# bytedance/monolith

Measured on AMD Instinct MI355X. Metric: embedding lookups+updates/sec at 1B ids x dim64, Zipf(1.2) batch=65536, higher is better.
Workload: dtype f32

## Files before the change

monolith_amd/csrc/mhte_step_kernels.h:

```cpp
#ifndef MHTE_STEP_KERNELS_H_
#define MHTE_STEP_KERNELS_H_

#include "mhte_kernels.h"

namespace mhte {

constexpr int kRdBlock = 1024;
constexpr int kRdLds = 2048;
constexpr int kRdStride = kRdLds + 1;
constexpr int kRdMaxBlocks = 64;
constexpr int kLongRun = kLightMax;
constexpr int kStepLightMax = 32;
constexpr int kMaxLongRuns = 16;
constexpr uint32_t kItemTarget = 256;
constexpr uint32_t kSpecSlackRows = 32;
#ifndef MHTE_BWD_OCC
#define MHTE_BWD_OCC 5
#endif
constexpr int kBwdBlocksPerCu = MHTE_BWD_OCC;

__device__ __forceinline__ void lds_barrier() {
  asm volatile("s_waitcnt lgkmcnt(0)\n\ts_barrier" ::: "memory");
}
__device__ __forceinline__ void lds_wave_sync() {
// ... 423 lines not shown
  uint32_t v = vt[ls];
  int left = kRdLds;
  while (k != id) {
    if (--left == 0) return 0u;
    ls = (ls + 1u) & (kRdLds - 1);
    k = kt[ls];
    v = vt[ls];
  }
  return v;
}

__device__ __forceinline__ uint32_t rd_find_run_opt(const RunView& d, uint32_t b, int64_t id) {
  const int64_t* kt = d.btab_key + size_t(b) * kRdStride;
  const uint32_t* vt = d.btab_val + size_t(b) * kRdStride;
  if (id == kEmptyKey) return run_cnt(vt[kRdLds]) ? vt[kRdLds] : 0u;
  uint32_t ls = rd_home(id);
  int64_t k = kt[ls];
  uint32_t v = vt[ls];
  int left = kRdLds;
  while (k != id) {
    if (k == kEmptyKey || --left == 0) return 0u;
    ls = (ls + 1u) & (kRdLds - 1);
    k = kt[ls];
    v = vt[ls];
  }
  return v;
}

__device__ __forceinline__ uint32_t rd_item_blocks(uint32_t c, uint32_t target) {
  uint32_t nbk = 64;
  const uint64_t lim = uint64_t(target) * 64 * (c > 2 * target ? 1 : 2);
  while (nbk > 1 && uint64_t(c) * nbk > lim) nbk >>= 1;
  return nbk;
}

constexpr int kBuildSlotsPerLane = 4;

constexpr int kMaxShards = 64;
__device__ __forceinline__ uint32_t shard_of_id(int64_t id, uint32_t nshards) {
  const int64_t m = id % int64_t(nshards);
  return uint32_t(m < 0 ? m + int64_t(nshards) : m);
}
struct PackCtl {
  int64_t* send_ids;
  const unsigned long long* peer_win;
  unsigned long long peer_ids_off;
  uint32_t* slot_off;
  uint32_t* flags;
  uint32_t world, ids_block, rows_block;
  uint32_t hdr_word;
  uint32_t cap, id_off, row_off, dim;
};

__device__ __forceinline__ void rd_emit_items(const RunView& d, int64_t id, uint32_t hu, uint32_t c,
                                              uint32_t hrow, uint32_t hspec, unsigned long long hloc,
                                              int lane) {
  const uint32_t val = (uint32_t(lane) < d.nblk) ? rd_find_run_opt(d, uint32_t(lane), id) : 0u;
  const unsigned long long bm = __ballot(val != 0u);
  const uint32_t nbk = rd_item_blocks(c, d.item_target);
  const uint32_t b0 = uint32_t(lane) & ~(nbk - 1u);
  const unsigned long long rmask = (nbk == 64 ? ~0ull : ((1ull << nbk) - 1ull)) << b0;
  const bool leader = (uint32_t(lane) == b0) && (bm & rmask) != 0ull;
  const unsigned long long lm = __ballot(leader);
  const uint32_t nitems = __popcll(lm);
  uint32_t w0 = 0;
  if (lane == 0) w0 = atomicAdd(&d.ctr[2], nitems);
  w0 = __shfl(w0, 0);
  const uint32_t k = __popcll(lm & ((1ull << b0) - 1ull));
  if (leader) {
    ItemHdr hd;
    hd.id = id;
    hd.u = hu;
    hd.meta = b0 | (nbk << 8) | (k << 16) | (nitems << 24);
    hd.row = hrow;
    hd.spec = hspec;
    hd.loc = hloc;
    d.item_hdr[w0 + k] = hd;
  }
  if ((bm & rmask) != 0ull) d.item_runs[size_t(w0 + k) * 64 + (uint32_t(lane) - b0)] = val;
}

constexpr unsigned long long kNoLoc = ~0ull;
struct __attribute__((aligned(16))) URec {
  int64_t id;
  uint32_t cnt;
  uint32_t pos;
  uint32_t slot;
  uint32_t row;
  unsigned long long loc;
};
struct ProbeOut {
  URec* urec;
  uint32_t reserve;
};

template <bool PACK = false, bool PROBE = false>
__device__ __forceinline__ void rd_build_role(const RunView& d, uint32_t light_max, uint32_t bid,
                                              uint32_t nblocks, const PackCtl* pc = nullptr,
                                              const TableView* tv = nullptr, ProbeOut po = ProbeOut{}) {
  constexpr int Q = kBuildSlotsPerLane;
  __shared__ uint32_t sh_tot[4];
  __shared__ uint32_t sh_base;
  __shared__ uint32_t sh_mtot[PROBE ? 4 : 1];
  __shared__ uint32_t sh_mbase;
  __shared__ uint8_t sh_stage[PROBE ? 4 * 256 : 4];
  __shared__ uint32_t sh_pc[PACK ? kMaxShards : 1], sh_pb[PACK ? kMaxShards : 1];
  const uint32_t t = threadIdx.x;
  const int lane = t & 63;
  const uint32_t nslots = d.cap_mask + 2u;
  for (uint32_t bb = bid * (256u * Q); bb < nslots; bb += nblocks * (256u * Q)) {
    const uint32_t base = bb + (t >> 6) * (64u * Q);
    int64_t key[Q];
    uint32_t cnt[Q], pos[Q];
    unsigned long long occ[Q];
    uint32_t total = 0;
    if (PACK) {
      if (t < pc->world) sh_pc[t] = 0;
      lds_barrier();
    }
#pragma unroll
    for (int q = 0; q < Q; ++q) {
      const uint32_t sl = base + q * 64 + lane;
      const bool in = sl < nslots;
      const RdSlot sv = d.hs[in ? sl : 0u];
      key[q] = in ? sv.key : kEmptyKey;
      cnt[q] = in ? uint32_t(sv.cp) : 0u;
      pos[q] = in ? uint32_t(sv.cp >> 32) : 0u;
    }
#pragma unroll
    for (int q = 0; q < Q; ++q) {
      const uint32_t sl = base + q * 64 + lane;
      const bool o = key[q] != kEmptyKey;
// ... 14 lines not shown
          prank[q] = atomicAdd(&sh_pc[pown[q]], 1u);
        }
      }
    }
    if (lane == 0) sh_tot[t >> 6] = total;
    lds_barrier();
    if (t == 0) {
      const uint32_t all = sh_tot[0] + sh_tot[1] + sh_tot[2] + sh_tot[3];
      sh_base = all ? atomicAdd(&d.ctr[0], all) : 0u;
    }
    if (PACK && t < pc->world) {
      const uint32_t c = sh_pc[t];
      sh_pb[t] = c ? uint32_t(atomicAdd(reinterpret_cast<unsigned long long*>(
                                            pc->send_ids + size_t(t) * pc->ids_block + pc->hdr_word),
                                        static_cast<unsigned long long>(c)))
                   : 0u;
    }
    lds_barrier();
    uint32_t k0 = sh_base;
    for (uint32_t w2 = 0; w2 < (t >> 6); ++w2) k0 += sh_tot[w2];
    const uint32_t kw0 = k0;
    const uint32_t wg_max = max(max(sh_tot[0], sh_tot[1]), max(sh_tot[2], sh_tot[3]));
    lds_barrier();
    uint32_t kq[Q];
#pragma unroll
    for (int q = 0; q < Q; ++q) {
      kq[q] = k0 + uint32_t(__popcll(occ[q] & ((1ull << lane) - 1ull)));
      k0 += uint32_t(__popcll(occ[q]));
      if ((occ[q] >> lane) & 1ull) {
        d.uids[kq[q]] = key[q];
        d.uslot[kq[q]] = base + q * 64 + lane;
        d.ucnt[kq[q]] = cnt[q];
        d.upos[kq[q]] = pos[q];
        if (PACK) {
          const uint32_t sl = sh_pb[pown[q]] + prank[q];
          if (sl < pc->cap) {
            if (pc->peer_win)
              reinterpret_cast<int64_t*>(pc->peer_win[pown[q]] + pc->peer_ids_off)[pc->id_off + sl] = key[q];
            else
              pc->send_ids[size_t(pown[q]) * pc->ids_block + pc->id_off + sl] = key[q];
            pc->slot_off[kq[q]] = pown[q] * pc->rows_block + pc->row_off + sl * pc->dim;
          } else {
            pc->slot_off[kq[q]] = 0xffffffffu;
            atomicOr(pc->flags, 1u);
          }
        }
      }
    }
    if (!PROBE) {
#pragma unroll
      for (int q = 0; q < Q; ++q) {
        unsigned long long hm = occ[q] & __ballot(cnt[q] > light_max);
        while (hm) {
          const int src = __ffsll(static_cast<long long>(hm)) - 1;
          hm &= hm - 1ull;
          rd_emit_items(d, __shfl(key[q], src), __shfl(kq[q], src), __shfl(cnt[q], src), kNoRow, kNoRow, 0ull,
                        lane);
        }
      }
    } else {
      typedef long long i64x2 __attribute__((ext_vector_type(2)));
      typedef unsigned int u32x4 __attribute__((ext_vector_type(4)));
      uint8_t* const stg = sh_stage + (t >> 6) * 256u;
      uint32_t run = 0;
#pragma unroll
      for (int q = 0; q < Q; ++q) {
        if ((occ[q] >> lane) & 1ull) stg[run + uint32_t(__popcll(occ[q] & ((1ull << lane) - 1ull)))] = uint8_t(q * 64 + lane);
        run += uint32_t(__popcll(occ[q]));
      }
      lds_wave_sync();
#pragma unroll 1
      for (uint32_t r0 = 0; r0 < wg_max; r0 += 64) {
        const uint32_t r = r0 + uint32_t(lane);
        const bool have = r < run;
        const uint32_t src = have ? uint32_t(stg[r]) : 0u;
        const int sl = int(src & 63u);
        int64_t kid = 0;
        uint32_t kc = 0, kp = 0;
#pragma unroll
        for (int q = 0; q < Q; ++q) {
          const int64_t kk = __shfl(key[q], sl);
          const uint32_t cc = __shfl(cnt[q], sl), pp = __shfl(pos[q], sl);
          if (int(src >> 6) == q) {
            kid = kk;
            kc = cc;
            kp = pp;
          }
        }
        const bool act = have && kid != kEmptyKey;
        const int64_t pid = act ? kid : 0;
        const uint64_t hv = hash_key(pid);
        const uint64_t i1 = index_hash(tv->hp, hv);
        const uint64_t i2 = alt_index(tv->hp, partial_key(hv), i1);
        const GBucket* b1 = global_bucket(tv->buckets + i1);
        const GBucket* b2 = global_bucket(tv->buckets + i2);
        const i64x2 k0a = *(const MHTE_GLOBAL i64x2*)(&b1->key[0]);
        const i64x2 k0b = *(const MHTE_GLOBAL i64x2*)(&b1->key[2]);
        const i64x2 k1a = *(const MHTE_GLOBAL i64x2*)(&b2->key[0]);
        const i64x2 k1b = *(const MHTE_GLOBAL i64x2*)(&b2->key[2]);
        const u32x4 r0v = *(const MHTE_GLOBAL u32x4*)(&b1->row[0]);
        const u32x4 r1v = *(const MHTE_GLOBAL u32x4*)(&b2->row[0]);
        int fs = -1;
        uint32_t fr = kNoRow;
        if (k1b.y == pid) { fs = 7; fr = r1v.w; }
        if (k1b.x == pid) { fs = 6; fr = r1v.z; }
        if (k1a.y == pid) { fs = 5; fr = r1v.y; }
        if (k1a.x == pid) { fs = 4; fr = r1v.x; }
        if (k0b.y == pid) { fs = 3; fr = r0v.w; }
        if (k0b.x == pid) { fs = 2; fr = r0v.z; }
        if (k0a.y == pid) { fs = 1; fr = r0v.y; }
        if (k0a.x == pid) { fs = 0; fr = r0v.x; }
        const bool found = act && fs >= 0 && fr != kNoRow;
        const bool miss = act && fs < 0;
        uint32_t spec = kNoRow;
        if (po.reserve) {
          const unsigned long long mm = __ballot(miss);
          if (lane == 0) sh_mtot[t >> 6] = uint32_t(__popcll(mm));
          lds_barrier();
          if (t == 0) {
            const unsigned long long all = sh_mtot[0] + sh_mtot[1] + sh_mtot[2] + sh_mtot[3];
            sh_mbase = all ? uint32_t(atomicAdd(&tv->ctr->alloc, (all << 32) | all)) : 0u;
            if (all) {
              atomicAdd(&tv->ctr->reserved, uint32_t(all));
              atomicAdd(&d.ctr[3], uint32_t(all));
            }
          }
          lds_barrier();
          uint32_t m0 = sh_mbase;
          for (uint32_t w2 = 0; w2 < (t >> 6); ++w2) m0 += sh_mtot[w2];
          lds_barrier();
          if (miss) spec = m0 + uint32_t(__popcll(mm & ((1ull << lane) - 1ull)));
        }
        const unsigned long long floc = found ? (((fs & 4) ? i2 : i1) << 2) | uint64_t(fs & 3) : kNoLoc;
        const uint32_t frow = found ? fr : spec;
        if (have) {
          URec rec;
          rec.id = kid;
          rec.cnt = kc;
          rec.pos = kp;
          rec.slot = base + (src >> 6) * 64u + (src & 63u);
          rec.row = frow;
          rec.loc = floc;
          po.urec[kw0 + r] = rec;
        }
        unsigned long long hm = __ballot(have && kc > light_max);
        while (hm) {
          const int s2 = __ffsll(static_cast<long long>(hm)) - 1;
          hm &= hm - 1ull;
          const unsigned long long hl = __shfl(floc, s2);
          rd_emit_items(d, __shfl(kid, s2), kw0 + r0 + uint32_t(s2), __shfl(kc, s2),
                        hl != kNoLoc ? __shfl(frow, s2) : kNoRow, hl != kNoLoc ? kNoRow : __shfl(frow, s2),
                        hl != kNoLoc ? hl : 0ull, lane);
        }
      }
    }
  }
  if (t == 0) {
    if (atomicAdd(&d.ctr[1], 1u) == nblocks - 1) *d.n_unique = atomicAdd(&d.ctr[0], 0u);
  }
}

__global__ __launch_bounds__(256) void rd_build_kernel(RunView d, uint32_t light_max) {
  rd_build_role(d, light_max, blockIdx.x, gridDim.x);
}
__global__ __launch_bounds__(256) void rd_build_probe_kernel(RunView d, uint32_t light_max, TableView tv,
                                                             ProbeOut po) {
  rd_build_role<false, true>(d, light_max, blockIdx.x, gridDim.x, nullptr, &tv, po);
}
__global__ __launch_bounds__(256) void rd_probe_kernel(RunView d, TableView tv, ProbeOut po, uint32_t n_max,
                                                       uint32_t light_max) {
  typedef long long i64x2 __attribute__((ext_vector_type(2)));
  typedef unsigned int u32x4 __attribute__((ext_vector_type(4)));
  __shared__ uint32_t sh_mtot[4];
  __shared__ uint32_t sh_mbase;
  const uint32_t t = threadIdx.x;
  const int lane = t & 63;
  const uint32_t nu = min(n_max, d.ctr[0]);
#pragma unroll 1
  for (uint32_t u0 = blockIdx.x * 256u; u0 < nu; u0 += gridDim.x * 256u) {
    const uint32_t u = u0 + t;
    const bool have = u < nu;
    const uint32_t us = have ? u : 0u;
    const int64_t kid = d.uids[us];
    const bool act = have && kid != kEmptyKey;
    const int64_t pid = act ? kid : 0;
    const uint64_t hv = hash_key(pid);
    const uint64_t i1 = index_hash(tv.hp, hv);
    const uint64_t i2 = alt_index(tv.hp, partial_key(hv), i1);
    const GBucket* b1 = global_bucket(tv.buckets + i1);
    const GBucket* b2 = global_bucket(tv.buckets + i2);
    const i64x2 k0a = *(const MHTE_GLOBAL i64x2*)(&b1->key[0]);
    const i64x2 k0b = *(const MHTE_GLOBAL i64x2*)(&b1->key[2]);
    const i64x2 k1a = *(const MHTE_GLOBAL i64x2*)(&b2->key[0]);
    const i64x2 k1b = *(const MHTE_GLOBAL i64x2*)(&b2->key[2]);
    const u32x4 r0v = *(const MHTE_GLOBAL u32x4*)(&b1->row[0]);
    const u32x4 r1v = *(const MHTE_GLOBAL u32x4*)(&b2->row[0]);
    URec rec;
    rec.id = kid;
    rec.cnt = d.ucnt[us];
    rec.pos = d.upos[us];
    rec.slot = d.uslot[us];
    int fs = -1;
    uint32_t fr = kNoRow;
    if (k1b.y == pid) { fs = 7; fr = r1v.w; }
    if (k1b.x == pid) { fs = 6; fr = r1v.z; }
// ... 99 lines not shown
  float* st2 = st1 + sd.dim;
  const bool has1 = sd.opt == kOptAdagrad || sd.opt == kOptFtrl;
  const bool has2 = sd.opt == kOptFtrl;
  Vec<VEC> s2;
  vec_zero(s2);
  if (is_new) {
    const SegDesc si = seg_for_init(sd);
#pragma unroll
    for (int c = 0; c < VEC; ++c) {
      r.w.v[c] = init_weight(si, rp + e + c);
      r.s1.v[c] = sd.p[0];
    }
  } else if (has2) {
    s2.load(st2);
  }
  if (sd.opt == kOptSgd) {
    const float slr = opaque_f(lr);
#pragma unroll
    for (int c = 0; c < VEC; ++c) r.w.v[c] = sgd_step(r.w.v[c], g.v[c], slr);
  } else if (sd.opt == kOptAdagrad) {
    const float alr = opaque_f(lr), wd = opaque_f(sd.p[1]);
    if (MHTE_AVX_FORM(sd)) {
#pragma unroll
      for (int c = 0; c < VEC; ++c)
        adagrad_step_avx(r.w.v[c], r.s1.v[c], g.v[c], alr, wd, uint32_t(le + c) < (uint32_t(sd.dim) & ~7u));
    } else {
#pragma unroll
      for (int c = 0; c < VEC; ++c) adagrad_step(r.w.v[c], r.s1.v[c], g.v[c], alr, wd);
    }
  } else {
    const float flr = opaque_f(lr), beta = opaque_f(sd.p[1]), l1 = opaque_f(sd.p[2]), l2 = opaque_f(sd.p[3]);
#pragma unroll
    for (int c = 0; c < VEC; ++c) ftrl_step(r.w.v[c], r.s1.v[c], s2.v[c], g.v[c], flr, beta, l1, l2);
  }
  row_store<VEC>(rp + e, r.w);
  if (has1) row_store<VEC>(st1, r.s1);
  if (has2) row_store<VEC>(st2, s2);
}

__device__ __forceinline__ void defer_id(const TableView& tv, uint32_t* pending, uint32_t u) {
  auto* ctr = tv.ctr;
#ifndef MHTE_NO_ANTIHOIST
  asm volatile("" : "+v"(ctr));
#endif
  pending[atomicAdd(&ctr->n_pending, 1u)] = u;
}

template <int G>
struct Probe {
  GBucket* b;
  int64_t k;
  uint32_t row;
};
template <int G>
__device__ __forceinline__ Probe<G> probe_issue(const TableView& tv, int64_t id, bool valid, int j) {
  const uint64_t hv = hash_key(id);
  const uint64_t i1 = index_hash(tv.hp, hv);
  const uint64_t i2 = alt_index(tv.hp, partial_key(hv), i1);
  Probe<G> p;
  p.b = global_bucket(tv.buckets + ((j < 4) ? i1 : i2));
  p.k = kEmptyKey;
  p.row = kNoRow;
  if (valid && id != kEmptyKey && j < 8) {
    p.k = p.b->key[j & 3];
    p.row = p.b->row[j & 3];
  }
  return p;
}

template <int VEC>
__device__ __forceinline__ void sum_list_lds(const float* __restrict__ grads, uint32_t dim,
                                             uint32_t e, bool ev, const uint32_t* pos, uint32_t c,
                                             Vec<VEC>& acc) {
#pragma unroll 1
  for (uint32_t q = 0; q < c; q += 8) {
    uint32_t ps[8];
#pragma unroll
    for (int t = 0; t < 8; ++t) ps[t] = (q + t < c) ? pos[q + t] : 0u;
    Vec<VEC> v[8];
#pragma unroll
    for (int t = 0; t < 8; ++t) vec_zero(v[t]);
#pragma unroll
    for (int t = 0; t < 8; ++t)
      if (q + t < c && ev) v[t].load(grads + int64_t(ps[t]) * dim + e);
#pragma unroll
    for (int t = 0; t < 8; ++t)
      if (q + t < c && ev) vec_add(acc, v[t]);
  }
}

template <int G>
struct UpsertFlight {
  unsigned long long cas_old;
  uint64_t specm;
  int owner, pick;
  bool found, need, special, deferred;
};

template <int G>
__device__ __forceinline__ UpsertFlight<G> upsert_issue(const TableView& tv, GBucket* b, int64_t id,
                                                        bool valid, int64_t k, int lane,
                                                        uint32_t reserved) {
  const int j = lane & (G - 1);
  const int gbase = lane & ~(G - 1);
  UpsertFlight<G> f;
  f.special = valid && id == kEmptyKey;
  const bool prober = valid && !f.special && j < 8;
  const uint64_t m = group_mask_of<G>(__ballot(prober && k == id), gbase);
  f.found = m != 0;
  f.owner = f.found ? (__ffsll(static_cast<long long>(m)) - 1) : -1;
  f.need = valid && !f.special && !f.found;
  f.deferred = false;
  const uint64_t em = group_mask_of<G>(__ballot(prober && k == kEmptyKey), gbase) & 0xffull;
  const uint32_t m1 = uint32_t(em) & 0xfu, m2 = (uint32_t(em) >> 4) & 0xfu;
  f.pick = -1;
  if (m1) f.pick = 31 - __clz(m1);
  else if (m2) f.pick = 4 + (31 - __clz(m2));
  if (f.need && f.pick < 0) {
    f.deferred = true;
    f.need = false;
  }
  f.cas_old = 0ull;
  if (f.need && j == f.pick)
    f.cas_old = cas_key(&b->key[j & 3], kEmptyKey, id);
  f.specm = __ballot(f.need && j == 0 && reserved == kNoRow);
  return f;
}

template <int G>
__device__ __forceinline__ SlotResult upsert_complete(const TableView& tv, GBucket* b, int64_t id,
                                                      bool valid, uint32_t row, int lane, uint32_t ts,
                                                      const UpsertFlight<G>& f, uint32_t base_row,
                                                      uint32_t reserved) {
  const int j = lane & (G - 1);
  const int gbase = lane & ~(G - 1);
  const int s = j & 3;
  const bool prober = valid && !f.special && j < 8;
  bool need = f.need, deferred = f.deferred, found = f.found, is_new = false;
  int owner = f.owner;
  int64_t k = 0;
  bool won = false;
  if (need && j == f.pick) {
    won = static_cast<int64_t>(f.cas_old) == kEmptyKey;
    k = won ? id : static_cast<int64_t>(f.cas_old);
  }
  {
    const uint64_t wm = group_mask_of<G>(__ballot(won), gbase);
    if (need && wm) {
      owner = f.pick;
      is_new = true;
      need = false;
    }
  }
  if (__any(need)) {
    if (prober) k = __hip_atomic_load(&b->key[s], __ATOMIC_RELAXED, __HIP_MEMORY_SCOPE_AGENT);
    while (__any(need)) {
      const uint64_t em = group_mask_of<G>(__ballot(prober && k == kEmptyKey), gbase) & 0xffull;
      int pick = -1;
      if (need) {
        const uint32_t m1 = uint32_t(em) & 0xfu, m2 = (uint32_t(em) >> 4) & 0xfu;
        if (m1) pick = 31 - __clz(m1);
        else if (m2) pick = 4 + (31 - __clz(m2));
        if (pick < 0) {
// ... 22 lines not shown
    found = true;
    is_new = (st == 0);
  }
  (void)found;
  const bool leader_new = is_new && j == 0;
  const uint64_t newm = __ballot(leader_new);
  const uint64_t resm = __ballot(valid && reserved != kNoRow && j == 0);
  const uint64_t extra = newm & ~f.specm & ~resm;
  const uint64_t lostm = (f.specm | resm) & ~newm;
  uint32_t base2 = 0;
  if (extra) {
    const int first2 = __ffsll(static_cast<long long>(extra)) - 1;
    if (lane == first2)
      base2 = static_cast<uint32_t>(
          atomicAdd(&tv.ctr->alloc, static_cast<unsigned long long>(__popcll(extra))));
    base2 = __shfl(base2, first2);
  }
  if (lostm && lane == __ffsll(static_cast<long long>(lostm)) - 1)
    atomicAdd(&tv.ctr->alloc, ~((static_cast<unsigned long long>(__popcll(lostm)) << 32) - 1ull));
  const uint32_t found_row = __shfl(row, gbase + (owner < 0 ? 0 : owner));
  int gb = gbase;
  asm volatile("" : "+v"(gb));
  const uint64_t below = (uint64_t(1) << gb) - 1;
  uint32_t r;
  if (is_new) {
    r = (reserved != kNoRow) ? reserved
        : ((f.specm >> gbase) & 1ull) ? base_row + uint32_t(__popcll(f.specm & below))
                                      : base2 + uint32_t(__popcll(extra & below));
  } else {
    r = found_row;
  }
  if (f.special) {
    auto* ctr = tv.ctr;
#ifndef MHTE_NO_ANTIHOIST
    asm volatile("" : "+v"(ctr));
#endif
    if (is_new) {
      if (j == 0) ctr->special_row = r;
    } else {
      r = ctr->special_row;
    }
    if (j == 0) ctr->special_ts = vgpr_copy_of_uniform(ts);
  } else if (valid && !deferred && j == owner) {
    if (is_new) b->row[s] = r;
    b->ts[s] = vgpr_copy_of_uniform(ts);
  }
  SlotResult out;
  out.r = r;
  out.is_new = is_new;
  out.deferred = deferred;
  return out;
}

struct ApplyLds {
  uint32_t pos[(256 / 8) * kStepLightMax];
  uint32_t rstart[65];
  uint32_t rval[64];
  float sum[256 * 4];
  uint32_t last;
};

template <int G, int VEC, bool ONESEG, bool HINT = false, bool FULL = false, int OPTK = -1, int FILT = -1>
__device__ __forceinline__ void rd_apply_role(const TableView& tv, const RunView& d,
                                              const ApplyCtl& c, const ApplyArgs& a, uint32_t bid,
                                              WaveTrace& wt, ApplyLds& L) {
  constexpr int WIN = G < 8 ? G : 8;
  constexpr int NG = 256 / G;
  const int lane = threadIdx.x & 63;
  const int j = lane & (G - 1);
  const int gbase = lane & ~(G - 1);
  const int grp = threadIdx.x / G;
  const uint32_t dim = tv.dim;
  const uint32_t e = uint32_t(j) * VEC;
  const bool ev = e < dim;

  if (bid >= c.nblk_items) {
    const uint32_t stride = c.nblk_ids * uint32_t(NG);
    const uint32_t k = bid - c.nblk_items;
    const uint32_t wave_s = __builtin_amdgcn_readfirstlane(threadIdx.x >> 6);
    uint32_t nu = c.n_max;
#pragma unroll 1
    for (uint32_t it = 0; uint64_t(it) * stride < nu; ++it) {
      uint32_t zero_ = 0;
      asm volatile("" : "+v"(zero_));
      const int lane = int(__builtin_amdgcn_mbcnt_hi(~0u, __builtin_amdgcn_mbcnt_lo(~0u, zero_)));
      const int j = lane & (G - 1);
      const int gbase = lane & ~(G - 1);
      const uint32_t e = uint32_t(j) * VEC;
      const bool ev = e < dim;
      const uint32_t grp_ = (uint32_t(wave_s) * 64u + uint32_t(lane)) / uint32_t(G);
      uint32_t* const sh_pos = L.pos + grp_ * kStepLightMax;
      const uint32_t g = it * stride + grp_ * c.nblk_ids + k;
      const bool inb = g < c.n_max;
      const uint32_t n_unique = d.ctr[0];
      int64_t id;
      uint32_t cnt, hp, gs, reserved = kNoRow, hrow = kNoRow, huts = 0;
      unsigned long long hloc = 0;
      if (!HINT) {
        const URec rec = c.urec[inb ? g : 0u];
        id = rec.id;
        cnt = inb ? rec.cnt : 0u;
        hp = rec.pos;
        gs = rec.slot;
        const bool fnd = rec.loc != kNoLoc;
        hrow = fnd ? rec.row : kNoRow;
        hloc = fnd ? rec.loc : 0ull;
        reserved = fnd ? kNoRow : rec.row;
      } else {
        reserved = kNoRow;
        id = inb ? d.uids[g] : 0;
        cnt = inb ? d.ucnt[g] : 0u;
        hp = inb ? d.upos[g] : 0u;
        gs = inb ? d.uslot[g] : 0u;
        if (c.urow) {
          hrow = inb ? c.urow[g] : kNoRow;
          hloc = inb ? c.uloc[g] : 0ull;
          if (c.uts) huts = inb ? c.uts[g] : 0u;
        }
      }
      const bool fgroup = FILT == 1 && tv.flt_slots != nullptr && tv.flt_nsplit != 0u;
// ... 89 lines not shown
          uint32_t first = 0;
          if constexpr (FILT == 1) {
            first = filter_consult_group<G>(tv, id, cnt, 2, contained, valid, fgroup && fact, fp, j, gbase, fhead,
                                            fhinc);
          } else {
            if (valid && j == 0) first = filter_consult(tv, id, cnt, 2, contained);
            first = __shfl(first, gbase);
          }
          if (first != 0u) valid = false;
          hinted = hinted && valid;
        }
      }
      const UpsertFlight<G> uf = upsert_issue<G>(tv, pr.b, id, valid && !hinted, pr.k, lane, reserved);
      const bool pre = valid && !hinted && uf.found;
      if (__any(pre)) {
        const uint32_t frow = __shfl(pr.row, gbase + (uf.owner < 0 ? 0 : uf.owner));
        if (pre && !FULL) row_prefetch<VEC, ONESEG>(tv, row_ptr(tv, frow), e, rr);
        if constexpr (PF) {
          if (pre) row_prefetch_full<VEC, OPTK>(tv, row_ptr(tv, frow), e, rf);
        }
      }
      if (__any(flat)) {
        uint32_t xr[PER];
#pragma unroll
        for (int q = 0; q < PER; ++q) xr[q] = 0;
#pragma unroll
        for (int q2 = 0; q2 < PER; ++q2) {
#pragma unroll 4
          for (int t2 = 0; t2 < G; ++t2) {
            const uint32_t y = __shfl(x[q2], gbase + t2);
#pragma unroll
            for (int q = 0; q < PER; ++q) xr[q] += (y < x[q]) ? 1u : 0u;
          }
        }
#pragma unroll
        for (int q = 0; q < PER; ++q)
          if (x[q] != 0xffffffffu) sh_pos[xr[q]] = x[q];
      }
      uint32_t rows0;
      bool bumped = false;
      {
        const unsigned long long tot = __popcll(uf.specm);
        if (tot && lane == 0) {
          rows0 = uint32_t(atomicAdd(&tv.ctr->alloc, (tot << 32) | tot));
          bumped = true;
        }
      }
      lds_wave_sync();
      if (it == 0) wt.mark(2);
      if (single) {
#pragma unroll
        for (int q = 0; q < VEC; ++q) acc.v[q] = 0.f + acc.v[q];
      }
      if (flat) sum_list_lds<VEC>(c.grads, dim, e, ev, sh_pos, cnt, acc);
      if (big) {
        unsigned long long rest = 0ull;
#pragma unroll 1
        for (uint32_t b1 = 0; b1 < d.nblk; b1 += G) {
          const uint32_t bq = b1 + uint32_t(j);
          const uint32_t vq = (bq < d.nblk) ? rd_find_run_opt(d, bq, id) : 0u;
          rest |= group_mask_of<G>(__ballot(vq != 0u), gbase) << b1;
        }
#pragma unroll 1
        while (rest) {
          const uint32_t b = uint32_t(__ffsll(static_cast<long long>(rest)) - 1);
          rest &= rest - 1ull;
          const uint32_t val = rd_find_run(d, b, id);
          const uint32_t cb = run_cnt(val);
          const uint16_t* sp = d.seg + b * kRdBlock + run_off(val);
#pragma unroll 1
          for (uint32_t i = 0; i < cb; i += 8) {
            Vec<VEC> v[8];
#pragma unroll
            for (int t = 0; t < 8; ++t) vec_zero(v[t]);
#pragma unroll
            for (int t = 0; t < 8; ++t)
              if (i + t < cb && ev)
                v[t].load(c.grads + int64_t(b * kRdBlock + sp[i + t]) * dim + e);
#pragma unroll
            for (int t = 0; t < 8; ++t)
              if (i + t < cb && ev) vec_add(acc, v[t]);
          }
        }
      }
      uint32_t base_row;
      {
        uint32_t br = bumped ? rows0 : 0u;
        base_row = __shfl(br, 0);
      }
      SlotResult sr =
          upsert_complete<G>(tv, pr.b, id, valid && !hinted, pr.row, lane, a.ts, uf, base_row, reserved);
      if (hinted) {
        sr.r = hrow;
        sr.is_new = false;
        sr.deferred = false;
        if (valid && j == 0 && !ts_known)
          global_bucket(tv.buckets + (hloc >> 2))->ts[hloc & 3ull] = vgpr_copy_of_uniform(a.ts);
      }
      float* rp = nullptr;
      if (valid && !sr.deferred) {
        rp = row_ptr(tv, sr.r);
        if (!FULL && !sr.is_new && !pre && !hinted) row_prefetch<VEC, ONESEG>(tv, rp, e, rr);
        if constexpr (PF) {
          if (!sr.is_new && !pre && !hinted) row_prefetch_full<VEC, OPTK>(tv, rp, e, rf);
        }
      }
      if (it == 0) wt.mark(3);
      if (sr.deferred) {
        if (ev) acc.store(c.grad_u + g * int64_t(dim) + e);
        if (j == 0) defer_id(tv, c.pending, uint32_t(g));
      } else if (valid) {
        if constexpr (PF) optimize_row_reg_full<VEC, ONESEG, OPTK>(tv, rp, sr.is_new, e, acc, a, &rf);
        else if (FULL) optimize_row_reg_full<VEC, ONESEG, OPTK>(tv, rp, sr.is_new, e, acc, a);
        else optimize_row_pre<VEC, ONESEG>(tv, rp, sr.is_new, e, acc, a, rr);
      }
      if (it == 0) wt.mark(4);
      lds_wave_sync();
    }
    return;
  }

  __builtin_amdgcn_s_setprio(3);
  uint32_t* const sh_rstart = L.rstart;
  uint32_t* const sh_rval = L.rval;
  float (*const sh_sum)[G * VEC] = reinterpret_cast<float (*)[G * VEC]>(L.sum);
  uint32_t& sh_last = L.last;
#pragma unroll 1
  for (uint32_t w = bid;; w += c.nblk_items) {
    const uint32_t nitems_all = d.ctr[2];
    const ItemHdr hd = d.item_hdr[w];
    const uint32_t rval = d.item_runs[size_t(w) * 64 + lane];
    asm volatile("" ::"v"(hd.meta), "v"(rval), "v"(nitems_all));
    if (w >= nitems_all) break;
    wt.mark(0);
    const uint32_t b0 = hd.meta & 0xffu, nbk = (hd.meta >> 8) & 0xffu, kk = (hd.meta >> 16) & 0xffu,
                   nitems = hd.meta >> 24;
    const bool ihint = hd.row != kNoRow;
    GBucket* const hb = global_bucket(tv.buckets + (hd.loc >> 2));
    int64_t vkey = hd.id;
    if (ihint && !c.trusted && threadIdx.x == 0) vkey = hb->key[hd.loc & 3ull];
    Probe<G> pr = probe_issue<G>(tv, hd.id, threadIdx.x < G && !ihint, j);
    const uint32_t reserved = threadIdx.x < G ? hd.spec : kNoRow;
    if (threadIdx.x < 64) {
      const uint32_t val = (uint32_t(lane) < nbk) ? rval : 0u;
      uint32_t incl = run_cnt(val);
#pragma unroll
      for (int o = 1; o < 64; o <<= 1) {
        const uint32_t v = __shfl_up(incl, o);
        if (lane >= o) incl += v;
      }
      sh_rval[lane] = val;
      sh_rstart[lane + 1] = incl;
      if (lane == 0) sh_rstart[0] = 0;
    }
    lds_barrier();
    wt.mark(1);
    const uint32_t E = c.pre_summed ? 0u : sh_rstart[64];
    Vec<VEC> acc;
    vec_zero(acc);
    constexpr int kPre = 2;
#pragma unroll 1
    for (uint32_t qb0 = uint32_t(grp) * WIN; qb0 < E; qb0 += kPre * NG * WIN) {
      constexpr int PPL = (kPre * WIN + G - 1) / G;
      uint32_t pp[PPL], pbv[PPL];
      uint16_t ps[PPL];
#pragma unroll
      for (int r = 0; r < PPL; ++r) {
        const uint32_t idx = uint32_t(r) * G + uint32_t(j);
        const uint32_t q = qb0 + (idx / WIN) * (NG * WIN) + (idx % WIN);
        const bool has = idx < uint32_t(kPre * WIN) && q < E;
        const uint32_t qq = has ? q : 0u;
        uint32_t lo = 0, hi = 63;
#pragma unroll
        for (int it2 = 0; it2 < 6; ++it2) {
          const uint32_t mid = (lo + hi + 1) >> 1;
          const bool le = sh_rstart[mid] <= qq;
          lo = le ? mid : lo;
          hi = le ? hi : mid - 1;
        }
        const uint32_t val = has ? sh_rval[lo] : 0u;
        const uint32_t base = (b0 + lo) * kRdBlock;
        ps[r] = d.seg[has ? base + run_off(val) + (qq - sh_rstart[lo]) : 0u];
        pbv[r] = base | (run_first(val) << 16) | ((run_cnt(val) == 1 ? 1u : 0u) << 31);
      }
#pragma unroll
      for (int r = 0; r < PPL; ++r)
        pp[r] = (pbv[r] & 0xffffu) + ((pbv[r] >> 31) ? ((pbv[r] >> 16) & 0x3ffu) : uint32_t(ps[r]));
#pragma unroll
      for (int w2 = 0; w2 < kPre; ++w2) {
        const uint32_t qb = qb0 + uint32_t(w2) * (NG * WIN);
        if (qb >= E) break;
        Vec<VEC> v[WIN];
#pragma unroll
        for (int t = 0; t < WIN; ++t) vec_zero(v[t]);
#pragma unroll
        for (int t = 0; t < WIN; ++t) {
          const int idx = w2 * WIN + t;
          const uint32_t pt = __shfl(pp[idx / G], gbase + (idx % G));
          if (qb + t < E && ev) v[t].load(c.grads + int64_t(pt) * dim + e);
        }
#pragma unroll
        for (int t = 0; t < WIN; ++t)
          if (qb + t < E && ev) vec_add(acc, v[t]);
      }
    }
#pragma unroll
    for (int cc = 0; cc < VEC; ++cc) sh_sum[grp][j * VEC + cc] = acc.v[cc];
    wt.mark(2);
    lds_barrier();
    Vec<VEC> tot;
    vec_zero(tot);
    if (threadIdx.x < 64) {
#pragma unroll 1
      for (int g2 = 0; g2 < NG; ++g2) {
#pragma unroll
        for (int cc = 0; cc < VEC; ++cc) tot.v[cc] = tot.v[cc] + sh_sum[g2][j * VEC + cc];
      }
    }
    wt.mark(3);
    bool apply = nitems == 1;
    if (c.pre_summed) {
      apply = kk == 0;
      if (apply && threadIdx.x < G && ev) tot.load(c.part + int64_t(w) * dim + e);
    } else if (nitems > 1) {
      if (threadIdx.x < G && ev) store_wt<VEC>(c.part + int64_t(w) * dim + e, tot);
      asm volatile("s_waitcnt vmcnt(0)" ::: "memory");
      lds_barrier();
      if (threadIdx.x == 0) {
        const uint32_t last = (atomicAdd(&c.arrive[hd.u], 1u) == nitems - 1) ? 1u : 0u;
        if (last) c.arrive[hd.u] = 0;
        sh_last = last;
      }
      lds_barrier();
      if (sh_last) {
        apply = true;
        const uint32_t w0 = w - kk;
        const uint32_t per = (nitems + NG - 1) / NG;
        const uint32_t k0 = min(nitems, uint32_t(grp) * per), k1 = min(nitems, k0 + per);
        Vec<VEC> sacc;
        vec_zero(sacc);
#pragma unroll 1
        for (uint32_t q = k0; q < k1; q += 8) {
          Vec<VEC> r[8];
#pragma unroll
          for (int t = 0; t < 8; ++t) vec_zero(r[t]);
#pragma unroll
          for (int t = 0; t < 8; ++t)
            if (q + t < k1 && ev) load_agent<VEC>(c.part + int64_t(w0 + q + t) * dim + e, r[t]);
#pragma unroll
          for (int t = 0; t < 8; ++t)
            if (q + t < k1 && ev) vec_add(sacc, r[t]);
        }
        lds_barrier();
#pragma unroll
        for (int cc = 0; cc < VEC; ++cc) sh_sum[grp][j * VEC + cc] = sacc.v[cc];
        lds_barrier();
        vec_zero(tot);
        if (threadIdx.x < 64) {
          for (int g2 = 0; g2 < NG && uint32_t(g2) * per < nitems; ++g2) {
#pragma unroll
            for (int cc = 0; cc < VEC; ++cc) tot.v[cc] = tot.v[cc] + sh_sum[g2][j * VEC + cc];
          }
        }
      }
    }
    if (apply && threadIdx.x < 64) {
      bool valid = threadIdx.x < G;
      bool hok = ihint && __shfl(vkey == hd.id ? 1 : 0, 0) != 0;
      if (ihint && !hok) pr = probe_issue<G>(tv, hd.id, valid, j);
      if constexpr (FILT != 0) {
        if (tv.flt_slots) {
          bool contained =
              group_mask_of<G>(__ballot(valid && hd.id != kEmptyKey && j < 8 && pr.k == hd.id), gbase) != 0;
          if (valid && hd.id == kEmptyKey) contained = tv.ctr->special_state == 1;
          if (hok) contained = true;
          uint32_t first = 0;
          if constexpr (FILT == 1) {
            uint32_t ih = 0, ii = 0;
            if (tv.flt_nsplit != 0u) {
              const FilterState* fs0 = reinterpret_cast<const FilterState*>(tv.flt_state);
              ih = fs0->head;
              ii = fs0->head_increment;
            }
            FilterProbe<G> fp0;
            first = filter_consult_group<G>(tv, hd.id, d.ucnt[hd.u], 2, contained, valid, false, fp0, j, gbase, ih, ii);
          } else {
            if (valid && j == 0) first = filter_consult(tv, hd.id, d.ucnt[hd.u], 2, contained);
            first = __shfl(first, gbase);
          }
          if (first != 0u) valid = false;
        }
      }
      SlotResult sr;
      if (hok) {
        sr.r = hd.row;
        sr.is_new = false;
        sr.deferred = false;
        if (valid && threadIdx.x == 0) hb->ts[hd.loc & 3ull] = vgpr_copy_of_uniform(a.ts);
      } else {
        sr = upsert_resolve<G>(tv, (Bucket*)pr.b, hd.id, valid, pr.k, pr.row, lane, vgpr_copy_of_uniform(a.ts),
                               reserved);
      }
      if (sr.deferred) {
        uint32_t ed = e;
#ifndef MHTE_NO_ANTIHOIST
        asm volatile("" : "+v"(ed));
#endif
        if (ev) tot.store(c.grad_u + int64_t(hd.u) * dim + ed);
        if (j == 0) defer_id(tv, c.pending, hd.u);
      } else if (valid) {
        if (FULL) optimize_row_reg_full<VEC, ONESEG, OPTK>(tv, row_ptr(tv, sr.r), sr.is_new, e, tot, a);
        else optimize_row_reg<VEC, ONESEG>(tv, row_ptr(tv, sr.r), sr.is_new, e, tot, a);
      }
    }
    wt.mark(4);
    lds_barrier();
  }
}

constexpr int kExactThreads = 512;
constexpr int kExactBufFloats = 16384;
constexpr int kExactMaxRows = 512;
struct __attribute__((aligned(16))) ExactLds {
  float buf[2][kExactBufFloats];
  uint32_t pos[3][kExactMaxRows];
  uint32_t rstart[65];
  uint32_t rbase[64];
};

template <int VEC, class DST>
__device__ __forceinline__ void rd_exact_sum_role(const RunView& d, const float* __restrict__ grads, uint32_t dim,
                                                  DST dst_of, uint32_t wg, uint32_t nwg, ExactLds& L) {
  constexpr uint32_t NL = kExactThreads - 64;
  const uint32_t t = threadIdx.x, lane = t & 63u;
  const uint32_t wave = __builtin_amdgcn_readfirstlane(t >> 6);
  const uint32_t C = min(uint32_t(kExactMaxRows), uint32_t(kExactBufFloats) / dim);
  const uint32_t upr = dim / VEC;
  const uint32_t nitems_all = d.ctr[2];
#pragma unroll 1
  for (uint32_t w = wg; w < nitems_all; w += nwg) {
    const ItemHdr hd = d.item_hdr[w];
    if (((hd.meta >> 16) & 0xffu) != 0u) continue;
    __syncthreads();
    if (wave == 0) {
      const uint32_t val = (lane < d.nblk) ? rd_find_run_opt(d, lane, hd.id) : 0u;
      uint32_t incl = run_cnt(val);
#pragma unroll
      for (int o = 1; o < 64; o <<= 1) {
        const uint32_t v = __shfl_up(incl, o);
        if (int(lane) >= o) incl += v;
      }
      L.rstart[lane + 1] = incl;
      if (lane == 0) L.rstart[0] = 0;
      L.rbase[lane] = lane * uint32_t(kRdBlock) + run_off(val);
    }
    __syncthreads();
    const uint32_t E = L.rstart[64];
    const uint32_t nch = (E + C - 1) / C;
    float acc[4] = {0.f, 0.f, 0.f, 0.f};
#pragma unroll 1
    for (int k = -2; k < int(nch); ++k) {
      if (wave != 0) {
        const uint32_t lt = t - 64u;
        const uint32_t c2 = uint32_t(k + 2);
        uint32_t pv[2] = {0u, 0u};
// ... 540 lines not shown
```

Measured before the change: 4.347 billion.

## Batch heavy-id item emission, add wave-wide list summing and LDS row prefetch

Several independent changes land together. Heavy ids are emitted in batches of four, with one atomic reservation per batch and interleaved hash-table lookups. Gradient-list summing now spreads long lists across idle lane groups within a wave. In the hinted apply path, embedding rows and optimizer state are DMA-prefetched into LDS via global_load_lds while partial sums accumulate. The alt-index hash and the owner-lane ffs are also tweaked. These aim to cut atomic traffic, load imbalance and row-load latency, at the cost of more registers, extra waitcnt barriers and added complexity.

```diff
diff --git a/monolith_amd/csrc/mhte_step_kernels.h b/monolith_amd/csrc/mhte_step_kernels.h
--- a/monolith_amd/csrc/mhte_step_kernels.h
+++ b/monolith_amd/csrc/mhte_step_kernels.h
@@ -499,32 +499,80 @@
   uint32_t cap, id_off, row_off, dim;
 };
 
-__device__ __forceinline__ void rd_emit_items(const RunView& d, int64_t id, uint32_t hu, uint32_t c,
-                                              uint32_t hrow, uint32_t hspec, unsigned long long hloc,
+#ifndef MHTE_EMIT_BATCH
+#define MHTE_EMIT_BATCH 4
+#endif
+constexpr int kEmitBatch = MHTE_EMIT_BATCH;
+struct HeavyId {
+  int64_t id;
+  uint32_t u, c, row, spec;
+  unsigned long long loc;
+};
+__device__ __forceinline__ uint32_t lane_value(uint32_t v, int src) {
+  return uint32_t(__builtin_amdgcn_readlane(int(v), src));
+}
+__device__ __forceinline__ unsigned long long lane_value64(unsigned long long v, int src) {
+  return (static_cast<unsigned long long>(lane_value(uint32_t(v >> 32), src)) << 32) | lane_value(uint32_t(v), src);
+}
+
+__device__ __forceinline__ void rd_emit_items(const RunView& d, const HeavyId (&h)[kEmitBatch], uint32_t nh,
                                               int lane) {
-  const uint32_t val = (uint32_t(lane) < d.nblk) ? rd_find_run_opt(d, uint32_t(lane), id) : 0u;
-  const unsigned long long bm = __ballot(val != 0u);
-  const uint32_t nbk = rd_item_blocks(c, d.item_target);
-  const uint32_t b0 = uint32_t(lane) & ~(nbk - 1u);
-  const unsigned long long rmask = (nbk == 64 ? ~0ull : ((1ull << nbk) - 1ull)) << b0;
-  const bool leader = (uint32_t(lane) == b0) && (bm & rmask) != 0ull;
-  const unsigned long long lm = __ballot(leader);
-  const uint32_t nitems = __popcll(lm);
+  const uint32_t bl = (uint32_t(lane) < d.nblk) ? uint32_t(lane) : 0u;
+  const int64_t* const kt = d.btab_key + size_t(bl) * kRdStride;
+  const uint32_t* const vt = d.btab_val + size_t(bl) * kRdStride;
+  uint32_t ls[kEmitBatch], v[kEmitBatch];
+  int64_t k[kEmitBatch];
+#pragma unroll
+  for (int i = 0; i < kEmitBatch; ++i) {
+    const int64_t id = h[uint32_t(i) < nh ? i : 0].id;
+    ls[i] = (id == kEmptyKey) ? uint32_t(kRdLds) : rd_home(id);
+    k[i] = kt[ls[i]];
+    v[i] = vt[ls[i]];
+  }
+  uint32_t nit[kEmitBatch], val[kEmitBatch], b0[kEmitBatch], kk[kEmitBatch];
+  bool leader[kEmitBatch], has[kEmitBatch];
+  uint32_t total = 0;
+#pragma unroll
+  for (int i = 0; i < kEmitBatch; ++i) {
+    const int64_t id = h[uint32_t(i) < nh ? i : 0].id;
+    int left = kRdLds;
+    while (k[i] != id && k[i] != kEmptyKey && --left != 0) {
+      ls[i] = (ls[i] + 1u) & (kRdLds - 1);
+      k[i] = kt[ls[i]];
+      v[i] = vt[ls[i]];
+    }
+    val[i] = (uint32_t(lane) < d.nblk && uint32_t(i) < nh && k[i] == id && run_cnt(v[i]) != 0u) ? v[i] : 0u;
+    const unsigned long long bm = __ballot(val[i] != 0u);
+    const uint32_t nbk = rd_item_blocks(h[i].c, d.item_target);
+    b0[i] = uint32_t(lane) & ~(nbk - 1u);
+    const unsigned long long rmask = (nbk == 64 ? ~0ull : ((1ull << nbk) - 1ull)) << b0[i];
+    has[i] = (bm & rmask) != 0ull;
+    leader[i] = (uint32_t(lane) == b0[i]) && has[i];
+    const unsigned long long lm = __ballot(leader[i]);
+    nit[i] = __popcll(lm);
+    kk[i] = __popcll(lm & ((1ull << b0[i]) - 1ull));
+    total += nit[i];
+  }
   uint32_t w0 = 0;
-  if (lane == 0) w0 = atomicAdd(&d.ctr[2], nitems);
+  if (lane == 0) w0 = atomicAdd(&d.ctr[2], total);
   w0 = __shfl(w0, 0);
-  const uint32_t k = __popcll(lm & ((1ull << b0) - 1ull));
-  if (leader) {
-    ItemHdr hd;
-    hd.id = id;
-    hd.u = hu;
-    hd.meta = b0 | (nbk << 8) | (k << 16) | (nitems << 24);
-    hd.row = hrow;
-    hd.spec = hspec;
-    hd.loc = hloc;
-    d.item_hdr[w0 + k] = hd;
-  }
-  if ((bm & rmask) != 0ull) d.item_runs[size_t(w0 + k) * 64 + (uint32_t(lane) - b0)] = val;
+#pragma unroll
+  for (int i = 0; i < kEmitBatch; ++i) {
+    if (uint32_t(i) < nh) {
+      if (leader[i]) {
+        ItemHdr hd;
+        hd.id = h[i].id;
+        hd.u = h[i].u;
+        hd.meta = b0[i] | (rd_item_blocks(h[i].c, d.item_target) << 8) | (kk[i] << 16) | (nit[i] << 24);
+        hd.row = h[i].row;
+        hd.spec = h[i].spec;
+        hd.loc = h[i].loc;
+        d.item_hdr[w0 + kk[i]] = hd;
+      }
+      if (has[i]) d.item_runs[size_t(w0 + kk[i]) * 64 + (uint32_t(lane) - b0[i])] = val[i];
+    }
+    w0 += nit[i];
+  }
 }
 
 constexpr unsigned long long kNoLoc = ~0ull;
@@ -645,10 +693,21 @@
       for (int q = 0; q < Q; ++q) {
         unsigned long long hm = occ[q] & __ballot(cnt[q] > light_max);
         while (hm) {
-          const int src = __ffsll(static_cast<long long>(hm)) - 1;
-          hm &= hm - 1ull;
-          rd_emit_items(d, __shfl(key[q], src), __shfl(kq[q], src), __shfl(cnt[q], src), kNoRow, kNoRow, 0ull,
-                        lane);
+          HeavyId h[kEmitBatch];
+          uint32_t nh = 0;
+#pragma unroll
+          for (int i = 0; i < kEmitBatch; ++i) {
+            const int src = hm ? __ffsll(static_cast<long long>(hm)) - 1 : 0;
+            nh += hm ? 1u : 0u;
+            hm &= hm - 1ull;
+            h[i].id = static_cast<int64_t>(lane_value64(static_cast<unsigned long long>(key[q]), src));
+            h[i].u = lane_value(kq[q], src);
+            h[i].c = lane_value(cnt[q], src);
+            h[i].row = kNoRow;
+            h[i].spec = kNoRow;
+            h[i].loc = 0ull;
+          }
+          rd_emit_items(d, h, nh, lane);
         }
       }
     } else {
@@ -738,12 +797,23 @@
         }
         unsigned long long hm = __ballot(have && kc > light_max);
         while (hm) {
-          const int s2 = __ffsll(static_cast<long long>(hm)) - 1;
-          hm &= hm - 1ull;
-          const unsigned long long hl = __shfl(floc, s2);
-          rd_emit_items(d, __shfl(kid, s2), kw0 + r0 + uint32_t(s2), __shfl(kc, s2),
-                        hl != kNoLoc ? __shfl(frow, s2) : kNoRow, hl != kNoLoc ? kNoRow : __shfl(frow, s2),
-                        hl != kNoLoc ? hl : 0ull, lane);
+          HeavyId h[kEmitBatch];
+          uint32_t nh = 0;
+#pragma unroll
+          for (int i = 0; i < kEmitBatch; ++i) {
+            const int s2 = hm ? __ffsll(static_cast<long long>(hm)) - 1 : 0;
+            nh += hm ? 1u : 0u;
+            hm &= hm - 1ull;
+            const unsigned long long hl = lane_value64(floc, s2);
+            const uint32_t hr = lane_value(frow, s2);
+            h[i].id = static_cast<int64_t>(lane_value64(static_cast<unsigned long long>(kid), s2));
+            h[i].u = kw0 + r0 + uint32_t(s2);
+            h[i].c = lane_value(kc, s2);
+            h[i].row = hl != kNoLoc ? hr : kNoRow;
+            h[i].spec = hl != kNoLoc ? kNoRow : hr;
+            h[i].loc = hl != kNoLoc ? hl : 0ull;
+          }
+          rd_emit_items(d, h, nh, lane);
         }
       }
     }
@@ -949,11 +1019,18 @@
   int64_t k;
   uint32_t row;
 };
+__device__ __forceinline__ uint64_t alt_index_tag(uint32_t hp, uint32_t partial, uint64_t index) {
+  uint32_t tag = partial + 1u;
+#ifndef MHTE_NO_ANTIHOIST
+  asm volatile("" : "+v"(tag));
+#endif
+  return (index ^ (uint64_t(tag) * 0xc6a4a7935bd1e995ULL)) & hash_mask(hp);
+}
 template <int G>
 __device__ __forceinline__ Probe<G> probe_issue(const TableView& tv, int64_t id, bool valid, int j) {
   const uint64_t hv = hash_key(id);
   const uint64_t i1 = index_hash(tv.hp, hv);
-  const uint64_t i2 = alt_index(tv.hp, partial_key(hv), i1);
+  const uint64_t i2 = alt_index_tag(tv.hp, partial_key(hv), i1);
   Probe<G> p;
   p.b = global_bucket(tv.buckets + ((j < 4) ? i1 : i2));
   p.k = kEmptyKey;
@@ -983,6 +1060,87 @@
 #pragma unroll
     for (int t = 0; t < 8; ++t)
       if (q + t < c && ev) vec_add(acc, v[t]);
+  }
+}
+
+template <int G, int VEC>
+__device__ __forceinline__ void sum_lists_wave(const float* __restrict__ grads, uint32_t dim, uint32_t e,
+                                               bool ev, const uint32_t* wpos, uint32_t mylen, int lane,
+                                               Vec<VEC>& acc) {
+  constexpr int NGW = 64 / G;
+  const uint32_t grp = uint32_t(lane) / uint32_t(G);
+  const int j = lane & (G - 1);
+  uint32_t len[NGW], pre[NGW + 1];
+  uint32_t idle = 0;
+  pre[0] = 0;
+#pragma unroll
+  for (int g = 0; g < NGW; ++g) {
+    len[g] = lane_value(mylen, g * G);
+    pre[g + 1] = pre[g] + (len[g] ? (len[g] - 1u) / 8u : 0u);
+    idle |= (len[g] == 0u ? 1u : 0u) << g;
+  }
+  const uint32_t total = pre[NGW];
+  const uint32_t nfree0 = uint32_t(__popc(idle));
+#pragma unroll 1
+  for (uint32_t r = 0;; ++r) {
+    const uint32_t xbase = r == 0 ? 0u : nfree0 + (r - 1u) * uint32_t(NGW);
+    if (r != 0 && xbase >= total) break;
+    const bool own = r == 0 && mylen != 0u;
+    const uint32_t x = r == 0 ? uint32_t(__popc(idle & ((1u << grp) - 1u))) : xbase + grp;
+    uint32_t o = 0;
+#pragma unroll
+    for (int g = 1; g < NGW; ++g) o += (x >= pre[g]) ? 1u : 0u;
+    uint32_t olen = len[0], opre = pre[0];
+#pragma unroll
+    for (int g = 1; g < NGW; ++g) {
+      olen = (o == uint32_t(g)) ? len[g] : olen;
+      opre = (o == uint32_t(g)) ? pre[g] : opre;
+    }
+    const bool lent = !own && x < total;
+    const uint32_t sg = own ? grp : o;
+    const uint32_t first = own ? 0u : 8u * (1u + x - opre);
+    const uint32_t rows = own ? min(8u, mylen) : (lent ? min(8u, olen - first) : 0u);
+    const uint32_t* ps = wpos + sg * uint32_t(kStepLightMax) + (rows ? first : 0u);
+    const MHTE_GLOBAL char* const gb = (const MHTE_GLOBAL char*)grads;
+    uint32_t pq[8];
+#pragma unroll
+    for (int t = 0; t < 8; ++t) pq[t] = (ps[t] * dim + e) * 4u;
+    Vec<VEC> v[8];
+#pragma unroll
+    for (int t = 0; t < 8; ++t) vec_zero(v[t]);
+#pragma unroll
+    for (int t = 0; t < 8; ++t)
+      if (uint32_t(t) < rows && ev) v[t].load((const float*)(gb + pq[t]));
+#pragma unroll
+    for (int t = 0; t < 8; ++t)
+      if (own && uint32_t(t) < rows && ev) vec_add(acc, v[t]);
+#pragma unroll 1
+    for (uint32_t sl = 0; sl < uint32_t(NGW); ++sl) {
+      if (r == 0 && ((idle >> sl) & 1u) == 0u) continue;
+      const uint32_t xs = r == 0 ? uint32_t(__popc(idle & ((1u << sl) - 1u))) : xbase + sl;
+      if (xs >= total) break;
+      uint32_t os = 0;
+#pragma unroll
+      for (int g = 1; g < NGW; ++g) os += (xs >= pre[g]) ? 1u : 0u;
+      uint32_t slen = len[0], spre = pre[0];
+#pragma unroll
+      for (int g = 1; g < NGW; ++g) {
+        slen = (os == uint32_t(g)) ? len[g] : slen;
+        spre = (os == uint32_t(g)) ? pre[g] : spre;
+      }
+      const uint32_t rs = min(8u, slen - 8u * (1u + xs - spre));
+      const int from = int(sl) * G + j;
+#pragma unroll
+      for (int t = 0; t < 8; ++t) {
+        if (uint32_t(t) < rs) {
+#pragma unroll
+          for (int cc = 0; cc < VEC; ++cc) {
+            const float y = __shfl(v[t].v[cc], from);
+            if (grp == os) acc.v[cc] = acc.v[cc] + y;
+          }
+        }
+      }
+    }
   }
 }
 
@@ -1005,7 +1163,7 @@
   const bool prober = valid && !f.special && j < 8;
   const uint64_t m = group_mask_of<G>(__ballot(prober && k == id), gbase);
   f.found = m != 0;
-  f.owner = f.found ? (__ffsll(static_cast<long long>(m)) - 1) : -1;
+  f.owner = f.found ? ((G <= 32 ? __ffs(int(uint32_t(m))) : __ffsll(static_cast<long long>(m))) - 1) : -1;
   f.need = valid && !f.special && !f.found;
   f.deferred = false;
   const uint64_t em = group_mask_of<G>(__ballot(prober && k == kEmptyKey), gbase) & 0xffull;
@@ -1134,8 +1292,32 @@
   return out;
 }
 
+template <int G>
+__device__ __forceinline__ void row_dma_issue(const TableView& tv, uint32_t row, int lane, float* dst) {
+  typedef const MHTE_GLOBAL void* gptr_t;
+  typedef __attribute__((address_space(3))) void* lptr_t;
+  const SegDesc sd = tv.seg[0];
+  const uint32_t el = uint32_t(lane & (G - 1)) * 4u;
+  const bool state = lane >= G;
+  const bool has1 = sd.opt == kOptAdagrad || sd.opt == kOptFtrl;
+  const float* rp = tv.chunk0 + size_t(row) * tv.row_floats;
+  const float* src = state ? rp + sd.st_off + (el - sd.w_off) : rp + el;
+  if (lane < 2 * G && el < tv.dim && (!state || has1))
+    __builtin_amdgcn_global_load_lds((gptr_t)src, (lptr_t)dst, 16, 0, 0);
+}
+template <int G, int VEC>
+__device__ __forceinline__ void row_from_lds(const float* src, int j, RowRegs<VEC>& r) {
+#pragma unroll
+  for (int c = 0; c < VEC; ++c) {
+    r.w.v[c] = src[j * VEC + c];
+    r.s1.v[c] = src[(G + j) * VEC + c];
+  }
+}
+
+constexpr int kRowDmaMaxG = 16;
 struct ApplyLds {
   uint32_t pos[(256 / 8) * kStepLightMax];
+  __attribute__((aligned(16))) float row[2 * kRowDmaMaxG * 4];
   uint32_t rstart[65];
   uint32_t rval[64];
   float sum[256 * 4];
@@ -1148,6 +1330,16 @@
                                               WaveTrace& wt, ApplyLds& L) {
   constexpr int WIN = G < 8 ? G : 8;
   constexpr int NG = 256 / G;
+#ifdef MHTE_NO_ROW_DMA
+  constexpr bool ROW_DMA = false;
+#else
+  constexpr bool ROW_DMA = !HINT && !FULL && FILT == 0 && ONESEG && VEC == 4 && G <= kRowDmaMaxG;
+#endif
+#ifdef MHTE_NO_WIDE_LISTS
+  constexpr bool WIDE = false;
+#else
+  constexpr bool WIDE = !HINT && !FULL && FILT == 0 && G < 64;
+#endif
   const int lane = threadIdx.x & 63;
   const int j = lane & (G - 1);
   const int gbase = lane & ~(G - 1);
@@ -1343,7 +1535,16 @@
 #pragma unroll
         for (int q = 0; q < VEC; ++q) acc.v[q] = 0.f + acc.v[q];
       }
-      if (flat) sum_list_lds<VEC>(c.grads, dim, e, ev, sh_pos, cnt, acc);
+      if constexpr (WIDE) {
+        if (__any(flat && cnt > 8u)) {
+          sum_lists_wave<G, VEC>(c.grads, dim, e, ev, L.pos + wave_s * uint32_t((64 / G) * kStepLightMax),
+                                 flat ? cnt : 0u, lane, acc);
+        } else if (flat) {
+          sum_list_lds<VEC>(c.grads, dim, e, ev, sh_pos, cnt, acc);
+        }
+      } else {
+        if (flat) sum_list_lds<VEC>(c.grads, dim, e, ev, sh_pos, cnt, acc);
+      }
       if (big) {
         unsigned long long rest = 0ull;
 #pragma unroll 1
@@ -1432,6 +1633,10 @@
     if (ihint && !c.trusted && threadIdx.x == 0) vkey = hb->key[hd.loc & 3ull];
     Probe<G> pr = probe_issue<G>(tv, hd.id, threadIdx.x < G && !ihint, j);
     const uint32_t reserved = threadIdx.x < G ? hd.spec : kNoRow;
+    const bool row_dma = ROW_DMA && ihint && !c.pre_summed && (hd.row >> tv.chunk_shift) == 0u;
+    if constexpr (ROW_DMA) {
+      if (row_dma && nitems == 1 && threadIdx.x < 64) row_dma_issue<G>(tv, hd.row, lane, L.row);
+    }
     if (threadIdx.x < 64) {
       const uint32_t val = (uint32_t(lane) < nbk) ? rval : 0u;
       uint32_t incl = run_cnt(val);
@@ -1498,6 +1703,9 @@
 #pragma unroll
     for (int cc = 0; cc < VEC; ++cc) sh_sum[grp][j * VEC + cc] = acc.v[cc];
     wt.mark(2);
+    if constexpr (ROW_DMA) {
+      if (row_dma && nitems == 1 && threadIdx.x < 64) asm volatile("s_waitcnt vmcnt(0)" ::: "memory");
+    }
     lds_barrier();
     Vec<VEC> tot;
     vec_zero(tot);
@@ -1530,6 +1738,9 @@
         const uint32_t k0 = min(nitems, uint32_t(grp) * per), k1 = min(nitems, k0 + per);
         Vec<VEC> sacc;
         vec_zero(sacc);
+        if constexpr (ROW_DMA) {
+          if (row_dma && threadIdx.x < 64) row_dma_issue<G>(tv, hd.row, lane, L.row);
+        }
 #pragma unroll 1
         for (uint32_t q = k0; q < k1; q += 8) {
           Vec<VEC> r[8];
@@ -1541,6 +1752,9 @@
 #pragma unroll
           for (int t = 0; t < 8; ++t)
             if (q + t < k1 && ev) vec_add(sacc, r[t]);
+        }
+        if constexpr (ROW_DMA) {
+          if (row_dma && threadIdx.x < 64) asm volatile("s_waitcnt vmcnt(0)" ::: "memory");
         }
         lds_barrier();
 #pragma unroll
@@ -1583,14 +1797,18 @@
         }
       }
       SlotResult sr;
+      int lane_a = lane;
+#ifndef MHTE_NO_ANTIHOIST
+      if constexpr (ROW_DMA) asm volatile("" : "+v"(lane_a));
+#endif
       if (hok) {
         sr.r = hd.row;
         sr.is_new = false;
         sr.deferred = false;
         if (valid && threadIdx.x == 0) hb->ts[hd.loc & 3ull] = vgpr_copy_of_uniform(a.ts);
       } else {
-        sr = upsert_resolve<G>(tv, (Bucket*)pr.b, hd.id, valid, pr.k, pr.row, lane, vgpr_copy_of_uniform(a.ts),
-                               reserved);
+        sr = upsert_resolve<G>(tv, (Bucket*)pr.b, hd.id, valid, pr.k, pr.row, ROW_DMA ? lane_a : lane,
+                               vgpr_copy_of_uniform(a.ts), reserved);
       }
       if (sr.deferred) {
         uint32_t ed = e;
@@ -1600,8 +1818,20 @@
         if (ev) tot.store(c.grad_u + int64_t(hd.u) * dim + ed);
         if (j == 0) defer_id(tv, c.pending, hd.u);
       } else if (valid) {
-        if (FULL) optimize_row_reg_full<VEC, ONESEG, OPTK>(tv, row_ptr(tv, sr.r), sr.is_new, e, tot, a);
-        else optimize_row_reg<VEC, ONESEG>(tv, row_ptr(tv, sr.r), sr.is_new, e, tot, a);
+        if (FULL) {
+          optimize_row_reg_full<VEC, ONESEG, OPTK>(tv, row_ptr(tv, sr.r), sr.is_new, e, tot, a);
+        } else if (ROW_DMA && row_dma && hok) {
+          uint32_t ea = e;
+#ifndef MHTE_NO_ANTIHOIST
+          asm volatile("" : "+v"(ea));
+#endif
+          RowRegs<VEC> rr;
+          row_from_lds<G, VEC>(L.row, int(ea / VEC), rr);
+          optimize_row_pre<VEC, ONESEG>(tv, assume_global(tv.chunk0 + size_t(hd.row) * tv.row_floats), false, ea, tot,
+                                        a, rr);
+        } else {
+          optimize_row_reg<VEC, ONESEG>(tv, row_ptr(tv, sr.r), sr.is_new, e, tot, a);
+        }
       }
     }
     wt.mark(4);
```

New measurement: 3.757 billion. 0.864x the previous value.
